# frankyeh/UNet-Studio

Hardware: AMD Instinct MI355X
Metric: voxels/sec 3D U-Net train step @128^3 bf16 (higher is better)
Workload: dtype bf16

## Files before the change

unet-studio_amd/csrc/engine.cpp:

```cpp
#include <hip/hip_runtime.h>

#include <algorithm>
#include <atomic>
#include <cmath>
#include <cstdio>
#include <cstring>
#include <functional>
#include <stdexcept>
#include <string>
#include <mutex>
#include <random>
#include <unordered_map>
#include <vector>

#include "../../include/unet_hip.h"
#include "conv_select.h"
#include "graph.hpp"
#include "kernels.h"

using namespace unet;

namespace {

thread_local std::string g_err;
// ... 729 lines not shown
            const bool defer = gflat && p.wz_job_of_op[i] >= 0 && !on_main;
            const bool own = p.wz_off[i] != SIZE_MAX && (defer || (op.kind == OP_CONV && p.conv[i].wgrad == Wgrad::mfma));
            {
            ProfScope pw(i, UNET_PROF_WGRAD, sb);
            conv_wgrad(p.conv[i].wgrad, op.kind == OP_CONVT, p.dtype, cg, sd, op.nsrc, gptr(t), gparams[op.weight], gparams[op.bias],
                       ws + (own ? p.wz_off[i] : p.wgrad_off), on_main ? s : sb, defer, on_main ? 0 : p.side_polite[i], nullptr);
            }
            if (defer) { wz_ran[p.wz_job_of_op[i]] = 1; ++wz_pending; }
            if (wz_pending >= 3) flush_wz(sb);
        };
        const int64_t hold_from = (int64_t)64 * 64 * 64, hold_below = (int64_t)32 * 32 * 32;
        std::vector<int> held;
        bool deep_seen = false;
        constexpr int fork_every = 3;
        std::vector<int> pending;
        auto issue_pending = [&]() {
            if (pending.empty()) return;
            fork();
            for (int h : pending) do_wgrad(h);
            pending.clear();
        };
        for (int i = (int)g.ops.size() - 1; i >= op_lo; --i) {
            const Op& op = g.ops[i];
            const bool dry = i >= op_hi;
            if (op.kind == OP_NORM) continue;
            if (op.kind == OP_EXPORT) {
                if (grad_outs && grad_outs[op.out_level] && g.tensors[op.src[0]].needs_grad) {
                    if (!dry) launch_export_bwd(p.dtype, grad_outs[op.out_level], dst_of(op.src[0]), g.tensors[op.src[0]].voxels(), s);
                    mark(op);
                }
                continue;
            }
            int t = op.dst;
            if ((op.kind == OP_CONV) && op.out_level >= 0) {
                if (!(grad_outs && grad_outs[op.out_level])) continue;
                if (p.conv[i].fwd == Fwd::head) {
                    DstGrad dgh = dst_of(op.src[0]);
                    ProfScope ph(dry ? -2 : i, UNET_PROF_OTHER, s);
                    if (!dry) {
                        const bool defer = sb != s && p.head_op_off[i] != SIZE_MAX;
                        char* hs = ws + (defer ? p.head_op_off[i] : p.head_off);
                        launch_head_bwd(p.dtype, geom(op), src(op.src[0]), grad_outs[op.out_level], nullptr, params[op.weight], dgh,
                                        gparams[op.weight], gparams[op.bias], hs, s, defer);
                        if (defer) { fork(); launch_head_bwd_reduce(geom(op), gparams[op.weight], gparams[op.bias], hs, sb); }
                    }
                    if (dgh.ptr) mark(op);
                    continue;
                }
                if (!dry) launch_import_grad(p.dtype, grad_outs[op.out_level], gptr(t), g.tensors[t].C, g.tensors[t].voxels(), 0, s);
                init[t] = 1;
            }
            if (!g.tensors[t].needs_grad || !init[t]) continue;
            bool first_fused = false;
            if (!dry && p.conv[i].wgrad == Wgrad::first_mfma && g.tensors[t].norm >= 0 && !g.tensors[op.src[0]].needs_grad && sb != s &&
                p.wz_off[i] != SIZE_MAX && g.tensors[t].C % 8 == 0)
                first_fused = !env().no_first_wgrad_fuse;
            {
                const bool has_norm = g.tensors[t].norm >= 0;
                const bool done = has_norm && norm_done[t];
                int rows = 0;
                if (done) norm_done[t] = 0;
                else if (has_norm) { if (bn_tensor == t) rows = bn_rows; bn_tensor = -1; }
                if (!dry) { ProfScope ps(i, UNET_PROF_NORM_BWD, s); if (!done) view_backward(t, params, gparams, first_fused, rows); }
            }
            switch (op.kind) {
                case OP_CONV:
                case OP_CONVT: {
                    SrcDesc sd[2] = {src(op.src[0]), op.nsrc > 1 ? src(op.src[1]) : SrcDesc()};
                    DstGrad dg[2] = {dst_of(op.src[0]), op.nsrc > 1 ? dst_of(op.src[1]) : DstGrad()};
                    ConvGeom cg = geom(op);
                    const float* wd = (const float*)(ws + p.w_dgrad[i]);
                    bool any = dg[0].ptr || (op.nsrc > 1 && dg[1].ptr);
                    if (!dry && !any && sb != s && p.conv[i].wgrad == Wgrad::first_mfma && p.wz_off[i] != SIZE_MAX) {
                        ProfScope pw(i, UNET_PROF_WGRAD, s);
                        const Tensor& To = g.tensors[t];
                        NormBwdFuse nf = {tptr(t), first_fused ? stat(To.norm) : nullptr, first_fused ? coef(To.norm) : nullptr, To.act};
                        conv_wgrad(p.conv[i].wgrad, false, p.dtype, cg, sd, op.nsrc, gptr(t), gparams[op.weight], gparams[op.bias], ws + p.wz_off[i],
                                   s, false, 0, first_fused ? &nf : nullptr);
                    } else
                    if (!dry) {
                        const int64_t vox = (int64_t)cg.Do * cg.Ho * cg.Wo;
                        if (!deep_seen && vox <= hold_below && !held.empty()) {
                            deep_seen = true;
                            pending.insert(pending.begin(), held.begin(), held.end());
                            held.clear();
                            pending.push_back(i);
                            issue_pending();
                        } else if (!deep_seen && sb != s && vox >= hold_from) held.push_back(i);
                        else {
                            pending.push_back(i);
                            if ((int)pending.size() >= fork_every || sb == s || vox >= hold_below) issue_pending();
                        }
                    }
                    ProfScope pd(i, UNET_PROF_DGRAD, s);
                    if (any) {
                        const int ts = op.src[0];
                        const Tensor& Ts = g.tensors[ts];
                        const bool can = op.nsrc == 1 && Ts.norm >= 0 && p.first_consumer[ts] == i && p.dtype == UNET_DTYPE_BF16;
                        DeepNormBwd nb;
                        if (can) {
                            const Norm& n = g.norms[Ts.norm];
                            nb = {tptr(ts), stat(Ts.norm), params[n.gamma], coef(Ts.norm), gparams[n.gamma], gparams[n.beta], Ts.act};
                        }
                        const DgradOutcome o = conv_dgrad(p.conv[i].dgrad, op.kind == OP_CONVT, p.dtype, cg, gptr(t), at(p.wm_dgrad[i]), wd, dg, op.nsrc,
                                                          can ? &nb : nullptr, partial(), deep(), s, !dry);
                        if (o.norm_done) norm_done[ts] = 1;
                        if (o.rows > 0) { bn_tensor = ts; bn_rows = o.rows; }
                        mark(op);
                    }
                    break;
                }
                case OP_MATERIALIZE: {
                    DstGrad dg[2] = {dst_of(op.src[0]), op.nsrc > 1 ? dst_of(op.src[1]) : DstGrad()};
                    if (dg[0].ptr || (op.nsrc > 1 && dg[1].ptr)) {
                        if (!dry) launch_materialize_bwd(p.dtype, gptr(t), dg, op.nsrc, g.tensors[t].voxels(), s);
                        mark(op);
                    }
                    break;
                }
                case OP_MAXPOOL: {
                    const Tensor& a = g.tensors[op.src[0]];
                    DstGrad d = dst_of(op.src[0]);
                    if (d.ptr) { if (!dry) launch_maxpool_bwd(p.dtype, src(op.src[0]), gptr(t), d, a.D, a.H, a.W, s); mark(op); }
                    break;
                }
                case OP_UPSAMPLE: {
                    const Tensor& a = g.tensors[op.src[0]];
                    DstGrad d = dst_of(op.src[0]);
                    if (d.ptr) { if (!dry) launch_upsample_bwd(p.dtype, gptr(t), d, a.D, a.H, a.W, s); mark(op); }
// ... 1905 lines not shown
```

unet-studio_amd/csrc/kernels.h:

```cpp
#pragma once
#include <hip/hip_runtime.h>
#include <cstdint>

#include "../../include/unet_atlas.h"
#include "../../include/unet_augment.h"
#include "../../include/unet_calib.h"
#include "../../include/unet_recal.h"
#include "../../include/unet_components.h"
#include "../../include/unet_connectivity.h"
#include "../../include/unet_distance.h"
#include "../../include/unet_ensemble.h"
#include "../../include/unet_feed.h"
#include "../../include/unet_hip.h"
#include "../../include/unet_instances.h"
#include "../../include/unet_morph.h"
#include "../../include/unet_postproc.h"
#include "../../include/unet_preproc.h"
#include "../../include/unet_qc.h"
#include "../../include/unet_register.h"
#include "../../include/unet_space.h"
#include "../../include/unet_stats.h"
#include "../../include/unet_table.h"
#include "../../include/unet_mirror.h"
#include "../../include/unet_tiles.h"
// ... 98 lines not shown
                     int* zero, int nzero, const float* partial, int nblk, float lr, float momentum, int nesterov, float weight_decay,
                     float clip_norm, float grad_scale, float* norm_out, hipStream_t s);

struct PackJob { int64_t src_off, dst_off, total, blk0; int Ci, Co, CK, T, mode, A, B, pad; };
enum PackMode {
    PK_CONV_FWD = 0,
    PK_CONV_DGRAD = 1,
    PK_CONVT_DGRAD = 2,
    PK_CONVT_FWD = 3,
    PK_CONV_S2_DGRAD = 4
};
int mfma_conv_pack_jobs(const ConvGeom& g, bool want_dgrad, PackJob* out2);
int mfma_convt_pack_jobs(const ConvGeom& g, PackJob* out2);
void launch_mfma_pack_batched(const float* params_base, void* ws, const PackJob* jobs_dev, int njobs, int64_t nblocks, hipStream_t s,
                              int64_t blk_base = 0, int max_grid = 0, int* zero = nullptr, int nzero = 0);
bool mfma_conv_fwd_supported(int dtype, const ConvGeom& g, const SrcDesc* src, int nsrc);
size_t mfma_conv_w_bytes(const ConvGeom& g);
void launch_mfma_pack_conv_w(const float* w, void* w_mfma_fwd, void* w_mfma_dgrad, const ConvGeom& g, hipStream_t s);
int launch_mfma_conv_fwd(const ConvGeom& g, const SrcDesc* src, int nsrc, const void* w_mfma, const float* bias, void* out,
                         float* stats_partial, hipStream_t s);
bool conv_first_mfma_supported(int dtype, const ConvGeom& g, const SrcDesc* src, int nsrc);
int conv_first_mfma_blocks(const ConvGeom& g);
int launch_conv_first_mfma(const ConvGeom& g, const SrcDesc* src, const float* w, const float* bias, void* out, float* stats_partial,
                           hipStream_t s);
int mfma_conv_blocks(const ConvGeom& g);
bool mfma_wgrad_z_supported(int dtype, const ConvGeom& g, const SrcDesc* src, int nsrc);
size_t mfma_wgrad_z_scratch_bytes(const ConvGeom& g, int polite = 0);
int mfma_wgrad_z_splits(const ConvGeom& g, int polite = 0);
int launch_mfma_wgrad_z(const ConvGeom& g, const SrcDesc* src, int nsrc, const void* dy, bool want_bias, void* scratch, hipStream_t s,
                        int polite = 0);
void wgrad_reduce(const float* slab, const float* bias_slab, int nsplit, int64_t n, int Cb, float* dw, float* db, hipStream_t s);
struct WgradReduceJob { long long slab_off, bias_off, dw_off, db_off, n; int nsplit, Cb, ly, blk0, nblk, op; };
int wgrad_reduce_job_blocks(WgradReduceJob& j, int blk0);
void launch_wgrad_reduce_batched(const WgradReduceJob* jobs_dev, int job0, int njobs, int blk_base, int nblocks, const void* ws, float* gflat,
                                 hipStream_t s);
bool mfma_wgrad_supported(int dtype, const ConvGeom& g, const SrcDesc* src, int nsrc);
size_t mfma_wgrad_scratch_bytes(const ConvGeom& g, int polite = 0);
int mfma_conv_wgrad_splits(const ConvGeom& g, int polite = 0);
int mfma_convt_wgrad_splits(const ConvGeom& g);
bool mfma_conv_wgrad_direct(const ConvGeom& g);
bool mfma_convt_wgrad_direct(const ConvGeom& g);
int conv_first_wgrad_splits(const ConvGeom& g);
void launch_mfma_conv_wgrad(const ConvGeom& g, const SrcDesc* src, int nsrc, const void* dy, float* dw, float* db, void* scratch,
                            hipStream_t s, bool defer_reduce = false, int polite = 0);
bool head_supported(const ConvGeom& g, int nsrc);
size_t head_bwd_scratch_bytes(const ConvGeom& g);
void launch_head_fwd(int dtype, const ConvGeom& g, const SrcDesc& src, const float* w, const float* bias, void* y, float* out_ncdhw,
                     hipStream_t s);
void launch_head_bwd(int dtype, const ConvGeom& g, const SrcDesc& src, const float* dy_ncdhw, const void* dy_cl, const float* w,
                     DstGrad dst, float* dw, float* db, void* scratch, hipStream_t s, bool defer_reduce = false);
void launch_head_bwd_reduce(const ConvGeom& g, float* dw, float* db, const void* scratch, hipStream_t s);
bool conv_first_wgrad_mfma_supported(int dtype, const ConvGeom& g, const SrcDesc* src, int nsrc);
size_t conv_first_wgrad_mfma_scratch_bytes(const ConvGeom& g);
struct NormBwdFuse { const void* u; const float* stat; const float* coef; int act; };
void launch_conv_first_wgrad_mfma(const ConvGeom& g, const SrcDesc* src, const void* dy, float* dw, float* db, void* scratch, hipStream_t s,
                                  bool defer_reduce = false, const NormBwdFuse* nb_fuse = nullptr);
bool wgrad_small_supported(const ConvGeom& g, int nsrc);
size_t wgrad_small_scratch_bytes(const ConvGeom& g);
void launch_conv_wgrad_small(int dtype, const ConvGeom& g, const SrcDesc* src, int nsrc, const void* dy, float* dw, float* db,
                             void* scratch, hipStream_t s);
bool mfma_convt_wgrad_supported(int dtype, const ConvGeom& g, const SrcDesc* src, int nsrc);
size_t mfma_convt_wgrad_scratch_bytes(const ConvGeom& g);
void launch_mfma_convt_wgrad(const ConvGeom& g, const SrcDesc* src, const void* dy, float* dw, void* scratch, hipStream_t s,
                             bool defer_reduce = false, float* db = nullptr, int polite = 0);
int launch_colsum_partial8(int dtype, const void* x, int C, int64_t S, float* partial, hipStream_t s);
size_t bias_grad_scratch_bytes(int C, int64_t S);
void launch_bias_grad(int dtype, const void* dy, int C, int64_t S, float* db, void* scratch, hipStream_t s);
bool mfma_conv_dgrad_supported(int dtype, const ConvGeom& g, const SrcDesc* src, int nsrc);
size_t mfma_conv_dgrad_w_bytes(const ConvGeom& g);
struct DgradOutcome {
    bool served = false;
    bool norm_done = false;
    int rows = 0;
    bool operator==(const DgradOutcome& o) const { return served == o.served && norm_done == o.norm_done && rows == o.rows; }
};
struct BnBwdStats { const void* u; const float* stat; float* partial; int act, C; };
DgradOutcome mfma_conv_dgrad_outcome(const ConvGeom& g, const DstGrad* dst, int ndst, bool norm);
DgradOutcome launch_mfma_conv_dgrad(const ConvGeom& g, const void* dy, const void* w_mfma_dgrad, const DstGrad* dst, int ndst, hipStream_t s,
                                    const BnBwdStats* bn = nullptr);
int launch_s2_conv_fwd(const ConvGeom& g, const SrcDesc* src, int nsrc, const void* w_mfma, const float* bias, void* out, float* stats_partial,
                       hipStream_t s);
DgradOutcome s2_conv_dgrad_outcome(const ConvGeom& g, const DstGrad* dst, int ndst, bool norm);
DgradOutcome launch_s2_conv_dgrad(const ConvGeom& g, const void* dy, const void* w_s2_dgrad, const DstGrad* dst, int ndst, hipStream_t s,
                                  const BnBwdStats* bn);
int s2_conv_dgrad_rows_max();
bool launch_s2_convt_fwd(const ConvGeom& g, const SrcDesc* src, int nsrc, const void* w_mfma, const float* bias, void* out, hipStream_t s);
bool launch_s2_convt_dgrad(const ConvGeom& g, const void* dy, const void* w_mfma_dgrad, const DstGrad* dst, int ndst, hipStream_t s);
int s2_wgrad_splits(int Ca, int Cb, int cD, int cH, int cW);
int launch_s2_wgrad(int ks, const void* fine, const void* fine2, int C0, int Ca, int fD, int fH, int fW, const void* coarse, int Cb, int cD, int cH,
                    int cW, bool want_bias, int bias_from_a, void* scratch, hipStream_t s, int polite);
constexpr int64_t DEEP_MAX_VOXELS = 512;
struct DeepScratch { float* part = nullptr; size_t part_bytes = 0; int* cnt = nullptr; int ncnt = 0; };
struct DeepNormFwd {
    const float* gamma; const float* beta; double eps; float* stat; float* rm; float* rv; double momentum; int use_running; int act;
    void* act_out;
};
struct DeepNormBwd {
    const void* u; const float* stat; const float* gamma; float* coef; float* dgamma; float* dbeta; int act;
};
bool deep_conv_applies(int dtype, int64_t out_voxels, int cin, int cout);
bool launch_deep_conv_fwd(const ConvGeom& g, const SrcDesc* src, int nsrc, const void* w_mfma, const float* bias, void* out,
                          const DeepNormFwd* nf, const DeepScratch& sc, hipStream_t s);
bool launch_deep_convt_fwd(const ConvGeom& g, const SrcDesc* src, int nsrc, const void* w_mfma, const float* bias, void* out,
                           const DeepScratch& sc, hipStream_t s);
DgradOutcome deep_dgrad_outcome(const ConvGeom& g, bool transposed, const DstGrad* dst, int ndst, bool norm, const DeepScratch& sc);
DgradOutcome launch_deep_dgrad(const ConvGeom& g, bool transposed, const void* dy, const void* w_mfma_dgrad, const DstGrad* dst, int ndst,
                               const DeepNormBwd* nb, const DeepScratch& sc, hipStream_t s);
// ... 160 lines not shown
```

unet-studio_amd/csrc/kernels_mfma_conv.hip:

```cpp
#include <type_traits>
#include <cstdlib>
#include "mfma_util.h"

namespace unet {

constexpr int PACK_LDS_ELEMS = 16 * (32 * 27 + 1);
template <int CK, int T, int MODE>
__device__ __forceinline__ void pack_unit_t(const float* __restrict__ w, __bf16* __restrict__ out, int unit, int Co, int A, int B, __bf16* lds) {
    constexpr int KSTEPS = CK == 32 ? T : (T + 1) / 2;
    const int NTT = Co / 16;
    const int q = unit / NTT, nt = unit % NTT, o0 = nt * 16;
    constexpr int RS = CK * T + 1;
    constexpr int n = 16 * CK * T, U = 8;
    for (int e0 = threadIdx.x; e0 < n; e0 += 256 * U) {
        float v[U];
        int dst[U];
#pragma unroll
        for (int u = 0; u < U; ++u) {
            const int e = e0 + u * 256;
            int r = 0, c = 0, t = 0;
            int64_t src = -1;
            if (e < n) {
                if constexpr (MODE == PK_CONV_FWD || MODE == PK_CONVT_DGRAD) {
                    const int Ax = MODE == PK_CONV_FWD ? A : B;
// ... 573 lines not shown
                    const float mean = a.bn_stat[c + r], rstd = a.bn_stat[a.bn_C + c + r];
                    const float dv = rr[r] * act_d(fmaf(uu[r], a.bn_stat[2 * a.bn_C + c + r], a.bn_stat[3 * a.bn_C + c + r]), a.bn_act);
                    s1[r] = dv; s2[r] = dv * ((uu[r] - mean) * rstd);
                }
            } else {
                s1[0] = r0; s1[1] = r1; s1[2] = r2; s1[3] = r3;
                s2[0] = r0 * r0; s2[1] = r1 * r1; s2[2] = r2 * r2; s2[3] = r3 * r3;
            }
        }
    }
    float* const srows = BNS ? a.bn_partial : a.stats;
    if (srows) {
        __syncthreads();
#pragma unroll
        for (int r = 0; r < 4; ++r) {
            float u = s1[r], v = s2[r];
#pragma unroll
            for (int m = 1; m < 16; m <<= 1) { u += __shfl_xor(u, m); v += __shfl_xor(v, m); }
            if (j == 0) { red[(wave * 16 + gq * 4 + r) * 2] = u; red[(wave * 16 + gq * 4 + r) * 2 + 1] = v; }
        }
        __syncthreads();
        if (tid < 16) {
            float u = 0.f, v = 0.f;
#pragma unroll
            for (int w = 0; w < 4; ++w) { u += red[(w * 16 + tid) * 2]; v += red[(w * 16 + tid) * 2 + 1]; }
            srows[((size_t)bid * g.Cout + nt0 * 16 + tid) * 2 + 0] = u;
            srows[((size_t)bid * g.Cout + nt0 * 16 + tid) * 2 + 1] = v;
        }
    }
}

struct ConvFirstArgs {
    ConvGeom g;
    const void* x;
    const float* w;
    const float* bias;
    void* out;
    float* stats;
    int tiles_x, tiles_y, tiles_z;
};
template <int NT>
__global__ void __launch_bounds__(256, 2) k_conv_first_mfma(ConvFirstArgs a) {
    constexpr int BZ = 4, BY = 8, BX = 16, HZ = BZ + 2, HY = BY + 2, HX = BX + 2, NV = HZ * HY * HX;
    constexpr int ITERS = (NV + 255) / 256;
    __shared__ unsigned short tile[NV + 8];
    __shared__ float red[4 * NT * 16 * 2];
    const ConvGeom& g = a.g;
    const int tid = threadIdx.x, wave = tid >> 6, lane = tid & 63, j = lane & 15, gq = lane >> 4;
    const int ntiles = a.tiles_x * a.tiles_y * a.tiles_z;
    const unsigned short* x = (const unsigned short*)a.x;

    bf16x8 wfrag[NT];
#pragma unroll
    for (int n = 0; n < NT; ++n)
#pragma unroll
        for (int e = 0; e < 8; ++e) {
            const int tap = 8 * gq + e;
            wfrag[n][e] = (__bf16)(tap < 27 ? a.w[(n * 16 + j) * 27 + tap] : 0.f);
        }
    int abase[8];
#pragma unroll
    for (int e = 0; e < 8; ++e) {
        const int tap = 8 * gq + e < 27 ? 8 * gq + e : 26;
        abase[e] = ((((tap / 9) + wave) * HY + (tap / 3) % 3) * HX + tap % 3 + j) * 2;
    }
    float b4[NT][4];
#pragma unroll
    for (int n = 0; n < NT; ++n)
#pragma unroll
        for (int r = 0; r < 4; ++r) b4[n][r] = a.bias ? a.bias[n * 16 + gq * 4 + r] : 0.f;
    float s1[NT][4], s2[NT][4];
#pragma unroll
    for (int n = 0; n < NT; ++n)
#pragma unroll
        for (int r = 0; r < 4; ++r) { s1[n][r] = 0.f; s2[n][r] = 0.f; }

    int upk[ITERS];
    unsigned uvox[ITERS];
#pragma unroll
    for (int k = 0; k < ITERS; ++k) {
        const int u = tid + k * 256, hz = u / (HY * HX), hr = u % (HY * HX), hy = hr / HX, hx = hr % HX;
        upk[k] = u < NV ? (hz | (hy << 4) | (hx << 9)) : -1;
        uvox[k] = (unsigned)((hz * g.H + hy) * g.W + hx);
    }
    unsigned short R[ITERS];
    auto prefetch = [&](int t) {
        const int x0 = (t % a.tiles_x) * BX, y0 = ((t / a.tiles_x) % a.tiles_y) * BY, z0 = (t / (a.tiles_x * a.tiles_y)) * BZ;
        const int iz0 = z0 - 1, iy0 = y0 - 1, ix0 = x0 - 1;
        const long long org = ((long long)iz0 * g.H + iy0) * g.W + ix0;
#pragma unroll
        for (int k = 0; k < ITERS; ++k) {
            const int uc = upk[k];
            const int gz = iz0 + (uc & 15), gy = iy0 + ((uc >> 4) & 31), gx = ix0 + ((uc >> 9) & 63);
            R[k] = 0;
            if (uc >= 0 && (unsigned)gz < (unsigned)g.D && (unsigned)gy < (unsigned)g.H && (unsigned)gx < (unsigned)g.W)
                R[k] = x[org + uvox[k]];
        }
    };
    if ((int)blockIdx.x < ntiles) prefetch(blockIdx.x);
    for (int t = blockIdx.x; t < ntiles; t += gridDim.x) {
        __syncthreads();
#pragma unroll
        for (int k = 0; k < ITERS; ++k)
            if (upk[k] >= 0) tile[tid + k * 256] = R[k];
        __syncthreads();
        if (t + (int)gridDim.x < ntiles) prefetch(t + gridDim.x);
        const int x0 = (t % a.tiles_x) * BX, y0 = ((t / a.tiles_x) % a.tiles_y) * BY, z0 = (t / (a.tiles_x * a.tiles_y)) * BZ;
        const int gz = z0 + wave, gx = x0 + j;
#pragma unroll
        for (int i = 0; i < BY; ++i) {
            unsigned d[4];
#pragma unroll
            for (int e = 0; e < 4; ++e) {
                const unsigned lo = *(const unsigned short*)((const char*)tile + abase[2 * e] + i * HX * 2);
                const unsigned hi = *(const unsigned short*)((const char*)tile + abase[2 * e + 1] + i * HX * 2);
                d[e] = lo | (hi << 16);
// ... 561 lines not shown
```

unet-studio_amd/csrc/kernels_mfma_wgrad.hip:

```cpp
#include <type_traits>
#include "mfma_util.h"

namespace unet {

typedef __attribute__((ext_vector_type(4))) short s16x4;
typedef __attribute__((address_space(3))) s16x4 lds_s16x4;

struct MfmaWgradArgs {
    ConvGeom g;
    SrcDesc asrc[2];
    int nasrc;
    SrcDesc bsrc;
    float* slab;
    float* bias_slab;
    int tiles_x, tiles_y, tiles_z;
    int direct;
    int bias_from_a;
};

__device__ __forceinline__ bf16x8 tr_read2(const char* p0, const char* p1) {
    s16x4 a = __builtin_amdgcn_ds_read_tr16_b64_v4i16((lds_s16x4*)p0);
    s16x4 b = __builtin_amdgcn_ds_read_tr16_b64_v4i16((lds_s16x4*)p1);
    return __builtin_bit_cast(bf16x8, __builtin_shufflevector(a, b, 0, 1, 2, 3, 4, 5, 6, 7));
}
// ... 386 lines not shown
    const long long n = jb.n, ntot = n + (hb ? jb.Cb : 0);
    const long long i = ((long long)((int)blockIdx.x + blk_base - jb.blk0) * LX + lx) * 4;
    double s0 = 0.0, s1 = 0.0, s2 = 0.0, s3 = 0.0;
    if (i < ntot) {
        const float* base = i < n ? ws + jb.slab_off + i : ws + jb.bias_off + (i - n);
        const long long stride = i < n ? n : jb.Cb;
        int k = ly;
        for (; k + 7 * LY < jb.nsplit; k += 8 * LY) {
            float4 v[8];
#pragma unroll
            for (int u = 0; u < 8; ++u) v[u] = *(const float4*)(base + (long long)(k + u * LY) * stride);
#pragma unroll
            for (int u = 0; u < 8; ++u) { s0 += v[u].x; s1 += v[u].y; s2 += v[u].z; s3 += v[u].w; }
        }
        for (; k < jb.nsplit; k += LY) {
            const float4 v = *(const float4*)(base + (long long)k * stride);
            s0 += v.x; s1 += v.y; s2 += v.z; s3 += v.w;
        }
    }
    if (LY > 1) {
        red[threadIdx.x][0] = s0; red[threadIdx.x][1] = s1; red[threadIdx.x][2] = s2; red[threadIdx.x][3] = s3;
        __syncthreads();
        if (ly == 0) {
            s0 = s1 = s2 = s3 = 0.0;
            for (int k = 0; k < LY; ++k) { s0 += red[k * LX + lx][0]; s1 += red[k * LX + lx][1]; s2 += red[k * LX + lx][2]; s3 += red[k * LX + lx][3]; }
        }
    }
    if (ly == 0 && i < ntot) {
        float* d = i < n ? gflat + jb.dw_off + i : gflat + jb.db_off + (i - n);
        d[0] += (float)s0; d[1] += (float)s1; d[2] += (float)s2; d[3] += (float)s3;
    }
}
int wgrad_reduce_job_blocks(WgradReduceJob& j, int blk0) {
    j.ly = j.nsplit > 64 ? 16 : (j.nsplit > 8 ? 4 : 1);
    const long long quads = (j.n + (j.bias_off >= 0 ? j.Cb : 0) + 3) / 4;
    const int lx = 256 / j.ly;
    j.blk0 = blk0;
    j.nblk = (int)((quads + lx - 1) / lx);
    return j.nblk;
}
void launch_wgrad_reduce_batched(const WgradReduceJob* jobs_dev, int job0, int njobs, int blk_base, int nblocks, const void* ws, float* gflat,
                                 hipStream_t s) {
    if (njobs <= 0 || nblocks <= 0) return;
    k_wgrad_reduce_batched<<<(unsigned)nblocks, 256, 0, s>>>(jobs_dev, job0, njobs, blk_base, (const float*)ws, gflat);
}

struct FirstWgradArgs {
    ConvGeom g;
    const void* x;
    const void* dy;
    float* slab;
    float* bslab;
    int tiles_x, tiles_y, tiles_z;
    const void* u;
    const float* stat;
    const float* coef;
    int act;
};
template <int NT, bool FUSE>
__global__ void __launch_bounds__(256, 2) k_wgrad_first_mfma(FirstWgradArgs a) {
    constexpr int TZ = 2, TY = 8, TX = 32, HZ = TZ + 2, HY = TY + 2, NROW = TZ * TY, CO = 16 * NT;
    constexpr int XCOPY = HZ * HY * TX;
    constexpr int VSB = CO * 2 + 4;
    constexpr int DY_OFF = 3 * XCOPY * 2;
    __shared__ __attribute__((aligned(16))) char sm[DY_OFF + NROW * TX * VSB + 16];
    const ConvGeom& g = a.g;
    const int tid = threadIdx.x, wave = tid >> 6, lane = tid & 63, j = lane & 15, gq = lane >> 4;
    const unsigned short* x = (const unsigned short*)a.x;
    const char* dyb = (const char*)a.dy;
    int abase[2];
    bool ones_row = false;
#pragma unroll
    for (int rt = 0; rt < 2; ++rt) {
        int tap = rt * 16 + j;
        if (tap == 27) ones_row = true;
        if (tap > 26) tap = 26;
        const int kz = tap / 9, ky = (tap / 3) % 3, kx = tap % 3;
        abase[rt] = (kx * XCOPY + (kz * HY + ky) * TX + gq * 8) * 2;
    }
    const bf16x8 ones = __builtin_bit_cast(bf16x8, make_uint4(0x3f803f80u, 0x3f803f80u, 0x3f803f80u, 0x3f803f80u));
    f32x4 acc[2][NT];
#pragma unroll
    for (int rt = 0; rt < 2; ++rt)
#pragma unroll
        for (int n = 0; n < NT; ++n) acc[rt][n] = f32x4{0.f, 0.f, 0.f, 0.f};
    const int ntiles = a.tiles_x * a.tiles_y * a.tiles_z;
    constexpr int XI = (HZ * HY * (TX + 2) + 255) / 256, DI = NROW * TX * (CO / 8) / 256;
    static_assert(NROW * TX * (CO / 8) % 256 == 0, "dy units per thread");
    unsigned short xr[XI];
    uint4 dr[DI], ur[FUSE ? DI : 1];
    unsigned dmask = 0;
    float cA[8], cB[8], cD[8], csc[8], csh[8];
    if constexpr (FUSE) {
        const int c0 = (tid % (CO / 8)) * 8;
#pragma unroll
        for (int e = 0; e < 8; ++e) {
            const int c = c0 + e;
            const float mean = a.stat[c], rstd = a.stat[CO + c];
            csc[e] = a.stat[2 * CO + c]; csh[e] = a.stat[3 * CO + c];
            cA[e] = a.coef[c];
            cB[e] = -a.coef[c] * rstd * a.coef[2 * CO + c];
            cD[e] = -a.coef[c] * (a.coef[CO + c] - mean * rstd * a.coef[2 * CO + c]);
        }
    }
    const char* ub = (const char*)a.u;
    auto gload = [&](int t) {
        const int x0 = (t % a.tiles_x) * TX, y0 = ((t / a.tiles_x) % a.tiles_y) * TY, z0 = (t / (a.tiles_x * a.tiles_y)) * TZ;
#pragma unroll
        for (int i = 0; i < XI; ++i) {
            const int e = tid + i * 256;
            const int hx = e % (TX + 2), r = e / (TX + 2), hy = r % HY, hz = r / HY;
            const int gz = z0 - 1 + hz, gy = y0 - 1 + hy, gx = x0 - 1 + hx;
            unsigned short v = 0;
            if (e < HZ * HY * (TX + 2) && (unsigned)gz < (unsigned)g.D && (unsigned)gy < (unsigned)g.H && (unsigned)gx < (unsigned)g.W)
                v = x[((size_t)gz * g.H + gy) * g.W + gx];
            xr[i] = v;
        }
#pragma unroll
        for (int i = 0; i < DI; ++i) {
            const int u = tid + i * 256;
            const int c8 = u % (CO / 8), vx = (u / (CO / 8)) % TX, row = u / ((CO / 8) * TX);
            const int gz = z0 + row / TY, gy = y0 + row % TY, gx = x0 + vx;
            uint4 v = make_uint4(0u, 0u, 0u, 0u), w = make_uint4(0u, 0u, 0u, 0u);
            const bool in = gz < g.D && gy < g.H && gx < g.W;
            const size_t off = ((((size_t)gz * g.H + gy) * g.W + gx) * CO + c8 * 8) * 2;
            if (in) v = *(const uint4*)(dyb + off);
            if constexpr (FUSE) {
                if (in) w = *(const uint4*)(ub + off);
                ur[i] = w;
                dmask = in ? (dmask | (1u << i)) : (dmask & ~(1u << i));
            }
            dr[i] = v;
        }
    };
    auto lstore = [&]() {
#pragma unroll
        for (int i = 0; i < XI; ++i) {
            const int e = tid + i * 256;
            if (e < HZ * HY * (TX + 2)) {
                const int hx = e % (TX + 2), r = e / (TX + 2), hy = r % HY, hz = r / HY;
#pragma unroll
                for (int sft = 0; sft < 3; ++sft) {
                    const int k = hx - sft;
                    if (k >= 0 && k < TX) *(unsigned short*)(sm + (sft * XCOPY + (hz * HY + hy) * TX + k) * 2) = xr[i];
                }
            }
        }
#pragma unroll
        for (int i = 0; i < DI; ++i) {
            const int u = tid + i * 256;
            const int c8 = u % (CO / 8), vx = (u / (CO / 8)) % TX, row = u / ((CO / 8) * TX);
            unsigned* d = (unsigned*)(sm + DY_OFF + (row * TX + vx) * VSB + c8 * 16);
            if constexpr (FUSE) {
                if ((dmask >> i) & 1u) {
                    const unsigned gu[4] = {dr[i].x, dr[i].y, dr[i].z, dr[i].w}, uu[4] = {ur[i].x, ur[i].y, ur[i].z, ur[i].w};
                    unsigned o[4];
#pragma unroll
                    for (int e = 0; e < 8; e += 2) {
                        const float g0 = __uint_as_float(gu[e / 2] << 16), g1 = __uint_as_float(gu[e / 2] & 0xffff0000u);
                        const float u0 = __uint_as_float(uu[e / 2] << 16), u1 = __uint_as_float(uu[e / 2] & 0xffff0000u);
                        const float r0 = fmaf(cA[e] * g0, act_d(fmaf(u0, csc[e], csh[e]), a.act), fmaf(cB[e], u0, cD[e]));
                        const float r1 = fmaf(cA[e + 1] * g1, act_d(fmaf(u1, csc[e + 1], csh[e + 1]), a.act), fmaf(cB[e + 1], u1, cD[e + 1]));
                        o[e / 2] = (unsigned)__bfloat16_as_ushort(__float2bfloat16(r0)) | ((unsigned)__bfloat16_as_ushort(__float2bfloat16(r1)) << 16);
                    }
                    dr[i] = make_uint4(o[0], o[1], o[2], o[3]);
                }
            }
            d[0] = dr[i].x; d[1] = dr[i].y; d[2] = dr[i].z; d[3] = dr[i].w;
        }
    };
    if ((int)blockIdx.x < ntiles) gload(blockIdx.x);
    for (int t = blockIdx.x; t < ntiles; t += gridDim.x) {
        __syncthreads();
        lstore();
        __syncthreads();
        if (t + (int)gridDim.x < ntiles) gload(t + gridDim.x);
#pragma unroll 1
        for (int row = wave; row < NROW; row += 4) {
            const int rz = row / TY, ry = row % TY;
            const int roff = (rz * HY + ry) * TX * 2;
            bf16x8 af[2];
#pragma unroll
            for (int rt = 0; rt < 2; ++rt) af[rt] = *(const bf16x8*)(sm + abase[rt] + roff);
            if (ones_row) af[1] = ones;
#pragma unroll
            for (int n = 0; n < NT; ++n) {
                unsigned d[4];
                const char* pb = sm + DY_OFF + (row * TX + gq * 8) * VSB + (n * 16 + j) * 2;
#pragma unroll
                for (int e = 0; e < 4; ++e) {
                    const unsigned lo = *(const unsigned short*)(pb + (2 * e) * VSB), hi = *(const unsigned short*)(pb + (2 * e + 1) * VSB);
                    d[e] = lo | (hi << 16);
                }
                const bf16x8 bf = __builtin_bit_cast(bf16x8, make_uint4(d[0], d[1], d[2], d[3]));
#pragma unroll
                for (int rt = 0; rt < 2; ++rt) acc[rt][n] = __builtin_amdgcn_mfma_f32_16x16x32_bf16(af[rt], bf, acc[rt][n], 0, 0, 0);
            }
        }
    }
    __syncthreads();
    float* red = (float*)sm;
#pragma unroll
    for (int rt = 0; rt < 2; ++rt)
#pragma unroll
        for (int n = 0; n < NT; ++n) *(f32x4*)(red + (((wave * 2 + rt) * NT + n) * 64 + lane) * 4) = acc[rt][n];
    __syncthreads();
    const int O = 27 * g.Cout;
    float* sl = a.slab + (size_t)blockIdx.x * O;
    for (int e = tid; e < 2 * NT * 256; e += 256) {
        float v = 0.f;
#pragma unroll
        for (int w = 0; w < 4; ++w) v += red[w * 2 * NT * 256 + e];
        const int reg = e & 3, l2 = (e >> 2) & 63, rn = e >> 8, n = rn % NT, rt = rn / NT;
        const int tap = rt * 16 + 4 * (l2 >> 4) + reg, co = n * 16 + (l2 & 15);
        if (tap < 27) sl[co * 27 + tap] = v;
        else if (tap == 27) a.bslab[(size_t)blockIdx.x * g.Cout + co] = v;
    }
}
bool conv_first_wgrad_mfma_supported(int dtype, const ConvGeom& g, const SrcDesc* src, int nsrc) {
    return dtype == 1 && nsrc == 1 && g.Cin == 1 && g.ks == 3 && g.stride == 1 && (g.Cout == 16 || g.Cout == 32) && !src[0].scale &&
           src[0].act == 0;
}
static int first_wgrad_blocks(const ConvGeom& g) {
    int tiles = ((g.W + 31) / 32) * ((g.H + 7) / 8) * ((g.D + 1) / 2);
    return tiles < 512 ? tiles : 512;
}
size_t conv_first_wgrad_mfma_scratch_bytes(const ConvGeom& g) { return (size_t)first_wgrad_blocks(g) * (27 * g.Cout + g.Cout) * 4 + 256; }
int conv_first_wgrad_splits(const ConvGeom& g) { return first_wgrad_blocks(g); }
void launch_conv_first_wgrad_mfma(const ConvGeom& g, const SrcDesc* src, const void* dy, float* dw, float* db, void* scratch, hipStream_t s,
                                  bool defer_reduce, const NormBwdFuse* nb_fuse) {
    FirstWgradArgs a;
    a.g = g; a.x = src[0].ptr; a.dy = dy; a.slab = (float*)scratch;
    a.u = nb_fuse ? nb_fuse->u : nullptr; a.stat = nb_fuse ? nb_fuse->stat : nullptr; a.coef = nb_fuse ? nb_fuse->coef : nullptr;
    a.act = nb_fuse ? nb_fuse->act : 0;
    a.tiles_x = (g.W + 31) / 32; a.tiles_y = (g.H + 7) / 8; a.tiles_z = (g.D + 1) / 2;
    const int nb = first_wgrad_blocks(g);
    const int64_t O = 27 * g.Cout;
    a.bslab = a.slab + (size_t)nb * O;
    if (nb_fuse) {
        if (g.Cout == 16) k_wgrad_first_mfma<1, true><<<nb, 256, 0, s>>>(a);
        else k_wgrad_first_mfma<2, true><<<nb, 256, 0, s>>>(a);
    } else {
        if (g.Cout == 16) k_wgrad_first_mfma<1, false><<<nb, 256, 0, s>>>(a);
        else k_wgrad_first_mfma<2, false><<<nb, 256, 0, s>>>(a);
    }
    if (!defer_reduce) wgrad_reduce(a.slab, db ? a.bslab : nullptr, nb, O, g.Cout, dw, db, s);
}

static bool chan16(const ConvGeom& g, const SrcDesc* src, int nsrc) {
    if (g.Cin % 16 || g.Cout % 16) return false;
    for (int s = 0; s < nsrc; ++s)
        if (src[s].C % 16 || src[s].scale || src[s].act) return false;
    return true;
}
bool mfma_wgrad_supported(int dtype, const ConvGeom& g, const SrcDesc* src, int nsrc) {
    return dtype == 1 && g.ks == 3 && (g.stride == 1 || g.stride == 2) && chan16(g, src, nsrc);
}
bool mfma_convt_wgrad_supported(int dtype, const ConvGeom& g, const SrcDesc* src, int nsrc) {
    return dtype == 1 && nsrc == 1 && chan16(g, src, nsrc);
}

struct WgradCfg { int bz, by, bx, pi, pj, nsplit, gy, direct, polite = 0; };
static bool wgrad_direct_cfg(int kind, int bD, int bH, int bW, WgradCfg& c) {
    if (bD != bH || bH != bW) return false;
    if (bW == 4) { c.bz = 4; c.by = 4; c.bx = 4; }
    else if (bW == 8 && kind == 0) { c.bz = 8; c.by = 8; c.bx = 8; }
    else if (bW == 8) { c.bz = 2; c.by = 8; c.bx = 8; }
    else return false;
    c.pi = c.pj = 1; c.nsplit = 1; c.direct = 1;
    return true;
}
static WgradCfg wgrad_cfg(int kind, int Ca, int Cb, int bD, int bH, int bW) {
    WgradCfg c;
    c.direct = 0;
    int cat = Ca / 16, cbt = Cb / 16;
    if (wgrad_direct_cfg(kind, bD, bH, bW, c)) { c.gy = cat * cbt; return c; }
    if (kind == 0) {
        c.pi = cat % 2 == 0 ? 2 : 1; c.pj = cbt % 2 == 0 ? 2 : 1;
        if (bW >= 12) { c.pi = 1; c.pj = 1; }
        if (bW >= 12) { c.bz = 2; c.by = 8; c.bx = 16; }
        else if (bW > 4) { c.bz = 4; c.by = 8; c.bx = 8; }
        else { c.bz = 4; c.by = 8; c.bx = 4; }
    } else {
        c.pi = 1; c.pj = cbt % 4 == 0 ? 4 : (cbt % 2 == 0 ? 2 : 1);
        if (bW >= 12) { c.bz = 2; c.by = 4; c.bx = 16; }
        else if (bW > 4) { c.bz = 2; c.by = 8; c.bx = 8; }
// ... 149 lines not shown
```

unet-studio_amd/csrc/mfma_util.h:

```cpp
#pragma once
#include <atomic>
#include <cstdint>
#include <cstdlib>

#include "device_util.h"

namespace unet {

inline void set_max_lds_once(std::atomic<uint64_t>& done, const void* fn, int bytes) {
    int dev = 0;
    (void)hipGetDevice(&dev);
    const uint64_t bit = 1ull << (dev & 63);
    if (done.load(std::memory_order_acquire) & bit) return;
    (void)hipFuncSetAttribute(fn, hipFuncAttributeMaxDynamicSharedMemorySize, bytes);
    done.fetch_or(bit, std::memory_order_release);
}

inline int polite_lds(int lds, int polite) {
    constexpr int want = 83000;
    return (polite && want > lds) ? want : lds;
}
inline bool sliding_window_off() {
    static const bool off = getenv("UNET_NO_SLIDING_WINDOW") != nullptr;
    return off;
}

typedef __attribute__((ext_vector_type(8))) __bf16 bf16x8;
typedef __attribute__((ext_vector_type(4))) float f32x4;

__device__ __forceinline__ unsigned pack_bf16x2(float lo, float hi) {
    return (unsigned)__bfloat16_as_ushort(__float2bfloat16(lo)) | ((unsigned)__bfloat16_as_ushort(__float2bfloat16(hi)) << 16);
}
__device__ __forceinline__ float bf_lo(unsigned w) { return __uint_as_float(w << 16); }
__device__ __forceinline__ float bf_hi(unsigned w) { return __uint_as_float(w & 0xffff0000u); }

__device__ __forceinline__ int xcd_remap(int b, int n) {
    int q = n >> 3, r = n & 7, x = b & 7;
    return (x < r ? x * (q + 1) : r * (q + 1) + (x - r) * q) + (b >> 3);
}

__device__ __forceinline__ uint4 transform8(uint4 v, bool xf, const float* sc, const float* sh, int act) {
    if (!(xf || act)) return v;
    unsigned wv[4] = {v.x, v.y, v.z, v.w};
#pragma unroll
    for (int e = 0; e < 4; ++e) {
        float lo = bf_lo(wv[e]), hi = bf_hi(wv[e]);
        if (xf) { lo = fmaf(lo, sc[2 * e], sh[2 * e]); hi = fmaf(hi, sc[2 * e + 1], sh[2 * e + 1]); }
        lo = act_f(lo, act); hi = act_f(hi, act);
        wv[e] = pack_bf16x2(lo, hi);
    }
    return make_uint4(wv[0], wv[1], wv[2], wv[3]);
}

struct MfmaConvArgs {
    ConvGeom g;
    SrcDesc src[2];
    int nsrc;
    const void* w;
    const float* bias;
    void* out[2];
    int outC[2];
    int out_acc[2];
    int nout;
    float* stats;
    int tiles_x, tiles_y, tiles_z;
    int sc_C;
    int oD, oH, oW;
    const void* bn_u = nullptr;
    const float* bn_stat = nullptr;
    float* bn_partial = nullptr;
    int bn_act = 0, bn_C = 0;
};

struct ZWork { int nseg, zlen, cols_x, cols_y; };
inline int z_split(ZWork& zw, int planes, int gy, int min_zlen) {
    const int cols = zw.cols_x * zw.cols_y;
    int want = 512 / gy;
    if (want < 1) want = 1;
    const int nseg = (want + cols - 1) / cols;
    int zlen = (planes + nseg - 1) / nseg;
    if (zlen < min_zlen) zlen = min_zlen;
    if (zlen > planes) zlen = planes;
    zw.nseg = (planes + zlen - 1) / zlen; zw.zlen = zlen;
    const int items = cols * zw.nseg;
    return items < want ? items : want;
}
int launch_conv_z16(const MfmaConvArgs& a, hipStream_t s);
// ... 7 lines not shown
```

Baseline: 824.1 million.

## Recompute first-conv pre-norm output inside fused wgrad instead of loading it

The fused first-layer weight-gradient kernel no longer reads the saved pre-normalization activation u from global memory. It recomputes u on the fly from the single-channel input halo already staged in shared memory, using an MFMA with the first conv's weights plus bias, then applies the norm/activation backward before writing dy to LDS. The goal is to cut global memory traffic for a large 128^3 multichannel tensor, paid for with extra MFMA work, more registers and reloaded loads. The fusion is now restricted to layers whose forward also uses the first_mfma path, and a staging structure with masked loads is added, though the stage count is 1.

New measurement: 825.8 million (median of 4 runs). No clear change (+0.2%).

```diff
diff --git a/unet-studio_amd/csrc/engine.cpp b/unet-studio_amd/csrc/engine.cpp
--- a/unet-studio_amd/csrc/engine.cpp
+++ b/unet-studio_amd/csrc/engine.cpp
@@ -805,7 +805,7 @@
             }
             if (!g.tensors[t].needs_grad || !init[t]) continue;
             bool first_fused = false;
-            if (!dry && p.conv[i].wgrad == Wgrad::first_mfma && g.tensors[t].norm >= 0 && !g.tensors[op.src[0]].needs_grad && sb != s &&
+            if (!dry && p.conv[i].wgrad == Wgrad::first_mfma && p.conv[i].fwd == Fwd::first_mfma && g.tensors[t].norm >= 0 && !g.tensors[op.src[0]].needs_grad && sb != s &&
                 p.wz_off[i] != SIZE_MAX && g.tensors[t].C % 8 == 0)
                 first_fused = !env().no_first_wgrad_fuse;
             {
@@ -827,7 +827,7 @@
                     if (!dry && !any && sb != s && p.conv[i].wgrad == Wgrad::first_mfma && p.wz_off[i] != SIZE_MAX) {
                         ProfScope pw(i, UNET_PROF_WGRAD, s);
                         const Tensor& To = g.tensors[t];
-                        NormBwdFuse nf = {tptr(t), first_fused ? stat(To.norm) : nullptr, first_fused ? coef(To.norm) : nullptr, To.act};
+                        NormBwdFuse nf = {params[op.weight], params[op.bias], first_fused ? stat(To.norm) : nullptr, first_fused ? coef(To.norm) : nullptr, To.act};
                         conv_wgrad(p.conv[i].wgrad, false, p.dtype, cg, sd, op.nsrc, gptr(t), gparams[op.weight], gparams[op.bias], ws + p.wz_off[i],
                                    s, false, 0, first_fused ? &nf : nullptr);
                     } else
diff --git a/unet-studio_amd/csrc/kernels.h b/unet-studio_amd/csrc/kernels.h
--- a/unet-studio_amd/csrc/kernels.h
+++ b/unet-studio_amd/csrc/kernels.h
@@ -174,7 +174,7 @@
 void launch_head_bwd_reduce(const ConvGeom& g, float* dw, float* db, const void* scratch, hipStream_t s);
 bool conv_first_wgrad_mfma_supported(int dtype, const ConvGeom& g, const SrcDesc* src, int nsrc);
 size_t conv_first_wgrad_mfma_scratch_bytes(const ConvGeom& g);
-struct NormBwdFuse { const void* u; const float* stat; const float* coef; int act; };
+struct NormBwdFuse { const float* w; const float* bias; const float* stat; const float* coef; int act; };
 void launch_conv_first_wgrad_mfma(const ConvGeom& g, const SrcDesc* src, const void* dy, float* dw, float* db, void* scratch, hipStream_t s,
                                   bool defer_reduce = false, const NormBwdFuse* nb_fuse = nullptr);
 bool wgrad_small_supported(const ConvGeom& g, int nsrc);
diff --git a/unet-studio_amd/csrc/kernels_mfma_conv.hip b/unet-studio_amd/csrc/kernels_mfma_conv.hip
--- a/unet-studio_amd/csrc/kernels_mfma_conv.hip
+++ b/unet-studio_amd/csrc/kernels_mfma_conv.hip
@@ -649,16 +649,11 @@
 
     bf16x8 wfrag[NT];
 #pragma unroll
-    for (int n = 0; n < NT; ++n)
-#pragma unroll
-        for (int e = 0; e < 8; ++e) {
-            const int tap = 8 * gq + e;
-            wfrag[n][e] = (__bf16)(tap < 27 ? a.w[(n * 16 + j) * 27 + tap] : 0.f);
-        }
+    for (int n = 0; n < NT; ++n) wfrag[n] = first_conv_wfrag(a.w, n, j, gq);
     int abase[8];
 #pragma unroll
     for (int e = 0; e < 8; ++e) {
-        const int tap = 8 * gq + e < 27 ? 8 * gq + e : 26;
+        const int tap = first_conv_tap(gq, e);
         abase[e] = ((((tap / 9) + wave) * HY + (tap / 3) % 3) * HX + tap % 3 + j) * 2;
     }
     float b4[NT][4];
diff --git a/unet-studio_amd/csrc/kernels_mfma_wgrad.hip b/unet-studio_amd/csrc/kernels_mfma_wgrad.hip
--- a/unet-studio_amd/csrc/kernels_mfma_wgrad.hip
+++ b/unet-studio_amd/csrc/kernels_mfma_wgrad.hip
@@ -462,11 +462,13 @@
     float* slab;
     float* bslab;
     int tiles_x, tiles_y, tiles_z;
-    const void* u;
+    const float* w;
+    const float* bias;
     const float* stat;
     const float* coef;
     int act;
 };
+constexpr int first_wgrad_stages(int nt, bool fuse) { return 1; }
 template <int NT, bool FUSE>
 __global__ void __launch_bounds__(256, 2) k_wgrad_first_mfma(FirstWgradArgs a) {
     constexpr int TZ = 2, TY = 8, TX = 32, HZ = TZ + 2, HY = TY + 2, NROW = TZ * TY, CO = 16 * NT;
@@ -497,53 +499,89 @@
     const int ntiles = a.tiles_x * a.tiles_y * a.tiles_z;
     constexpr int XI = (HZ * HY * (TX + 2) + 255) / 256, DI = NROW * TX * (CO / 8) / 256;
     static_assert(NROW * TX * (CO / 8) % 256 == 0, "dy units per thread");
-    unsigned short xr[XI];
-    uint4 dr[DI], ur[FUSE ? DI : 1];
-    unsigned dmask = 0;
-    float cA[8], cB[8], cD[8], csc[8], csh[8];
+    constexpr int MT = (NROW / 4) * (TX / 16);
+    constexpr int NST = first_wgrad_stages(NT, FUSE);
+    struct Stage {
+        unsigned short xr[XI];
+        uint4 dr[FUSE ? 1 : DI];
+        uint2 gr[FUSE ? MT * NT : 1];
+        unsigned xmask, dmask;
+    };
+    Stage st[NST];
+    float cA[NT][4], cB[NT][4], cD[NT][4], csc[NT][4], csh[NT][4], b4[NT][4];
+    bf16x8 wfrag[NT];
+    int ubase[8];
     if constexpr (FUSE) {
-        const int c0 = (tid % (CO / 8)) * 8;
+#pragma unroll
+        for (int n = 0; n < NT; ++n) {
+            wfrag[n] = first_conv_wfrag(a.w, n, j, gq);
+#pragma unroll
+            for (int r = 0; r < 4; ++r) {
+                const int c = n * 16 + gq * 4 + r;
+                const float mean = a.stat[c], rstd = a.stat[CO + c];
+                csc[n][r] = a.stat[2 * CO + c]; csh[n][r] = a.stat[3 * CO + c];
+                cA[n][r] = a.coef[c];
+                cB[n][r] = -a.coef[c] * rstd * a.coef[2 * CO + c];
+                cD[n][r] = -a.coef[c] * (a.coef[CO + c] - mean * rstd * a.coef[2 * CO + c]);
+                b4[n][r] = a.bias ? a.bias[c] : 0.f;
+            }
+        }
 #pragma unroll
         for (int e = 0; e < 8; ++e) {
-            const int c = c0 + e;
-            const float mean = a.stat[c], rstd = a.stat[CO + c];
-            csc[e] = a.stat[2 * CO + c]; csh[e] = a.stat[3 * CO + c];
-            cA[e] = a.coef[c];
-            cB[e] = -a.coef[c] * rstd * a.coef[2 * CO + c];
-            cD[e] = -a.coef[c] * (a.coef[CO + c] - mean * rstd * a.coef[2 * CO + c]);
-        }
-    }
-    const char* ub = (const char*)a.u;
-    auto gload = [&](int t) {
+            const int tap = first_conv_tap(gq, e);
+            ubase[e] = ((tap % 3) * XCOPY + ((tap / 9) * HY + (tap / 3) % 3) * TX + j) * 2;
+        }
+    }
+    auto gload = [&](Stage& q, int t) {
+        const bool tv = t < ntiles;
         const int x0 = (t % a.tiles_x) * TX, y0 = ((t / a.tiles_x) % a.tiles_y) * TY, z0 = (t / (a.tiles_x * a.tiles_y)) * TZ;
+        unsigned xm = 0, dm = 0;
 #pragma unroll
         for (int i = 0; i < XI; ++i) {
             const int e = tid + i * 256;
             const int hx = e % (TX + 2), r = e / (TX + 2), hy = r % HY, hz = r / HY;
             const int gz = z0 - 1 + hz, gy = y0 - 1 + hy, gx = x0 - 1 + hx;
-            unsigned short v = 0;
-            if (e < HZ * HY * (TX + 2) && (unsigned)gz < (unsigned)g.D && (unsigned)gy < (unsigned)g.H && (unsigned)gx < (unsigned)g.W)
-                v = x[((size_t)gz * g.H + gy) * g.W + gx];
-            xr[i] = v;
-        }
-#pragma unroll
-        for (int i = 0; i < DI; ++i) {
-            const int u = tid + i * 256;
-            const int c8 = u % (CO / 8), vx = (u / (CO / 8)) % TX, row = u / ((CO / 8) * TX);
-            const int gz = z0 + row / TY, gy = y0 + row % TY, gx = x0 + vx;
-            uint4 v = make_uint4(0u, 0u, 0u, 0u), w = make_uint4(0u, 0u, 0u, 0u);
-            const bool in = gz < g.D && gy < g.H && gx < g.W;
-            const size_t off = ((((size_t)gz * g.H + gy) * g.W + gx) * CO + c8 * 8) * 2;
-            if (in) v = *(const uint4*)(dyb + off);
-            if constexpr (FUSE) {
-                if (in) w = *(const uint4*)(ub + off);
-                ur[i] = w;
-                dmask = in ? (dmask | (1u << i)) : (dmask & ~(1u << i));
-            }
-            dr[i] = v;
-        }
+            const bool in = tv && e < HZ * HY * (TX + 2) && (unsigned)gz < (unsigned)g.D && (unsigned)gy < (unsigned)g.H && (unsigned)gx < (unsigned)g.W;
+            const size_t idx = in ? ((size_t)gz * g.H + gy) * g.W + gx : (size_t)0;
+            q.xr[i] = x[idx];
+            xm |= (in ? 1u : 0u) << i;
+        }
+        if constexpr (FUSE) {
+#pragma unroll
+            for (int m = 0; m < MT; ++m) {
+                const int row = wave + 4 * (m / (TX / 16)), vx = (m % (TX / 16)) * 16 + j;
+                const int gz = z0 + row / TY, gy = y0 + row % TY, gx = x0 + vx;
+                const bool in = tv && gz < g.D && gy < g.H && gx < g.W;
+                const size_t off = in ? ((((size_t)gz * g.H + gy) * g.W + gx) * CO + gq * 4) * 2 : (size_t)0;
+#pragma unroll
+                for (int n = 0; n < NT; ++n) q.gr[m * NT + n] = *(const uint2*)(dyb + off + (in ? n * 32 : 0));
+                dm |= (in ? 1u : 0u) << m;
+            }
+        } else {
+#pragma unroll
+            for (int i = 0; i < DI; ++i) {
+                const int u = tid + i * 256;
+                const int c8 = u % (CO / 8), vx = (u / (CO / 8)) % TX, row = u / ((CO / 8) * TX);
+                const int gz = z0 + row / TY, gy = y0 + row % TY, gx = x0 + vx;
+                const bool in = tv && gz < g.D && gy < g.H && gx < g.W;
+                const size_t off = in ? ((((size_t)gz * g.H + gy) * g.W + gx) * CO + c8 * 8) * 2 : (size_t)0;
+                q.dr[i] = *(const uint4*)(dyb + off);
+                dm |= (in ? 1u : 0u) << i;
+            }
+        }
+        q.xmask = xm; q.dmask = dm;
     };
-    auto lstore = [&]() {
+    auto prep = [&](Stage& q) {
+#pragma unroll
+        for (int i = 0; i < XI; ++i)
+            if (!((q.xmask >> i) & 1u)) q.xr[i] = 0;
+        if constexpr (!FUSE) {
+#pragma unroll
+            for (int i = 0; i < DI; ++i)
+                if (!((q.dmask >> i) & 1u)) q.dr[i] = make_uint4(0u, 0u, 0u, 0u);
+        }
+    };
+    auto lstore = [&](const Stage& q) {
 #pragma unroll
         for (int i = 0; i < XI; ++i) {
             const int e = tid + i * 256;
@@ -552,39 +590,54 @@
 #pragma unroll
                 for (int sft = 0; sft < 3; ++sft) {
                     const int k = hx - sft;
-                    if (k >= 0 && k < TX) *(unsigned short*)(sm + (sft * XCOPY + (hz * HY + hy) * TX + k) * 2) = xr[i];
-                }
-            }
-        }
-#pragma unroll
-        for (int i = 0; i < DI; ++i) {
-            const int u = tid + i * 256;
-            const int c8 = u % (CO / 8), vx = (u / (CO / 8)) % TX, row = u / ((CO / 8) * TX);
-            unsigned* d = (unsigned*)(sm + DY_OFF + (row * TX + vx) * VSB + c8 * 16);
-            if constexpr (FUSE) {
-                if ((dmask >> i) & 1u) {
-                    const unsigned gu[4] = {dr[i].x, dr[i].y, dr[i].z, dr[i].w}, uu[4] = {ur[i].x, ur[i].y, ur[i].z, ur[i].w};
-                    unsigned o[4];
-#pragma unroll
-                    for (int e = 0; e < 8; e += 2) {
-                        const float g0 = __uint_as_float(gu[e / 2] << 16), g1 = __uint_as_float(gu[e / 2] & 0xffff0000u);
-                        const float u0 = __uint_as_float(uu[e / 2] << 16), u1 = __uint_as_float(uu[e / 2] & 0xffff0000u);
-                        const float r0 = fmaf(cA[e] * g0, act_d(fmaf(u0, csc[e], csh[e]), a.act), fmaf(cB[e], u0, cD[e]));
-                        const float r1 = fmaf(cA[e + 1] * g1, act_d(fmaf(u1, csc[e + 1], csh[e + 1]), a.act), fmaf(cB[e + 1], u1, cD[e + 1]));
-                        o[e / 2] = (unsigned)__bfloat16_as_ushort(__float2bfloat16(r0)) | ((unsigned)__bfloat16_as_ushort(__float2bfloat16(r1)) << 16);
-                    }
-                    dr[i] = make_uint4(o[0], o[1], o[2], o[3]);
-                }
-            }
-            d[0] = dr[i].x; d[1] = dr[i].y; d[2] = dr[i].z; d[3] = dr[i].w;
+                    if (k >= 0 && k < TX) *(unsigned short*)(sm + (sft * XCOPY + (hz * HY + hy) * TX + k) * 2) = q.xr[i];
+                }
+            }
+        }
+        if constexpr (!FUSE) {
+#pragma unroll
+            for (int i = 0; i < DI; ++i) {
+                const int u = tid + i * 256;
+                const int c8 = u % (CO / 8), vx = (u / (CO / 8)) % TX, row = u / ((CO / 8) * TX);
+                unsigned* d = (unsigned*)(sm + DY_OFF + (row * TX + vx) * VSB + c8 * 16);
+                d[0] = q.dr[i].x; d[1] = q.dr[i].y; d[2] = q.dr[i].z; d[3] = q.dr[i].w;
+            }
         }
     };
-    if ((int)blockIdx.x < ntiles) gload(blockIdx.x);
-    for (int t = blockIdx.x; t < ntiles; t += gridDim.x) {
-        __syncthreads();
-        lstore();
-        __syncthreads();
-        if (t + (int)gridDim.x < ntiles) gload(t + gridDim.x);
+    auto produce = [&](const Stage& q) {
+#pragma unroll
+        for (int m = 0; m < MT; ++m) {
+            const int row = wave + 4 * (m / (TX / 16)), vx0 = (m % (TX / 16)) * 16;
+            const int poff = (((row / TY) * HY + row % TY) * TX + vx0) * 2;
+            unsigned d[4];
+#pragma unroll
+            for (int e = 0; e < 4; ++e) {
+                const unsigned lo = *(const unsigned short*)(sm + ubase[2 * e] + poff), hi = *(const unsigned short*)(sm + ubase[2 * e + 1] + poff);
+                d[e] = lo | (hi << 16);
+            }
+            const bf16x8 xfrag = __builtin_bit_cast(bf16x8, make_uint4(d[0], d[1], d[2], d[3]));
+            const bool in = (q.dmask >> m) & 1u;
+#pragma unroll
+            for (int n = 0; n < NT; ++n) {
+                const f32x4 uacc = __builtin_amdgcn_mfma_f32_16x16x32_bf16(wfrag[n], xfrag, f32x4{0.f, 0.f, 0.f, 0.f}, 0, 0, 0);
+                const unsigned up[2] = {pack_bf16x2(uacc[0] + b4[n][0], uacc[1] + b4[n][1]), pack_bf16x2(uacc[2] + b4[n][2], uacc[3] + b4[n][3])};
+                const uint2 gv = q.gr[m * NT + n];
+                const unsigned gp[2] = {gv.x, gv.y};
+                unsigned o[2];
+#pragma unroll
+                for (int h = 0; h < 2; ++h) {
+                    const float g0 = bf_lo(gp[h]), g1 = bf_hi(gp[h]), u0 = bf_lo(up[h]), u1 = bf_hi(up[h]);
+                    const int r = 2 * h;
+                    const float r0 = fmaf(cA[n][r] * g0, act_d(fmaf(u0, csc[n][r], csh[n][r]), a.act), fmaf(cB[n][r], u0, cD[n][r]));
+                    const float r1 = fmaf(cA[n][r + 1] * g1, act_d(fmaf(u1, csc[n][r + 1], csh[n][r + 1]), a.act), fmaf(cB[n][r + 1], u1, cD[n][r + 1]));
+                    o[h] = in ? pack_bf16x2(r0, r1) : 0u;
+                }
+                unsigned* dst = (unsigned*)(sm + DY_OFF + (row * TX + vx0 + j) * VSB + (n * 16 + gq * 4) * 2);
+                dst[0] = o[0]; dst[1] = o[1];
+            }
+        }
+    };
+    auto compute = [&]() {
 #pragma unroll 1
         for (int row = wave; row < NROW; row += 4) {
             const int rz = row / TY, ry = row % TY;
@@ -606,6 +659,28 @@
 #pragma unroll
                 for (int rt = 0; rt < 2; ++rt) acc[rt][n] = __builtin_amdgcn_mfma_f32_16x16x32_bf16(af[rt], bf, acc[rt][n], 0, 0, 0);
             }
+        }
+    };
+    const int G = gridDim.x;
+#pragma unroll
+    for (int s = 0; s < NST; ++s) gload(st[s], (int)blockIdx.x + s * G);
+    prep(st[0]);
+    for (int t0 = blockIdx.x; t0 < ntiles; t0 += NST * G) {
+#pragma unroll
+        for (int s = 0; s < NST; ++s) {
+            const int t = t0 + s * G;
+            if (t < ntiles) {
+                __syncthreads();
+                lstore(st[s]);
+                __syncthreads();
+                if constexpr (FUSE) {
+                    produce(st[s]);
+                    __builtin_amdgcn_wave_barrier();
+                }
+            }
+            gload(st[s], t + NST * G);
+            if (t < ntiles) compute();
+            if (t + G < ntiles) prep(st[(s + 1) % NST]);
         }
     }
     __syncthreads();
@@ -641,7 +716,8 @@
                                   bool defer_reduce, const NormBwdFuse* nb_fuse) {
     FirstWgradArgs a;
     a.g = g; a.x = src[0].ptr; a.dy = dy; a.slab = (float*)scratch;
-    a.u = nb_fuse ? nb_fuse->u : nullptr; a.stat = nb_fuse ? nb_fuse->stat : nullptr; a.coef = nb_fuse ? nb_fuse->coef : nullptr;
+    a.w = nb_fuse ? nb_fuse->w : nullptr; a.bias = nb_fuse ? nb_fuse->bias : nullptr;
+    a.stat = nb_fuse ? nb_fuse->stat : nullptr; a.coef = nb_fuse ? nb_fuse->coef : nullptr;
     a.act = nb_fuse ? nb_fuse->act : 0;
     a.tiles_x = (g.W + 31) / 32; a.tiles_y = (g.H + 7) / 8; a.tiles_z = (g.D + 1) / 2;
     const int nb = first_wgrad_blocks(g);
diff --git a/unet-studio_amd/csrc/mfma_util.h b/unet-studio_amd/csrc/mfma_util.h
--- a/unet-studio_amd/csrc/mfma_util.h
+++ b/unet-studio_amd/csrc/mfma_util.h
@@ -33,6 +33,17 @@
 }
 __device__ __forceinline__ float bf_lo(unsigned w) { return __uint_as_float(w << 16); }
 __device__ __forceinline__ float bf_hi(unsigned w) { return __uint_as_float(w & 0xffff0000u); }
+
+__device__ __forceinline__ int first_conv_tap(int gq, int e) { return 8 * gq + e < 27 ? 8 * gq + e : 26; }
+__device__ __forceinline__ bf16x8 first_conv_wfrag(const float* __restrict__ w, int n, int j, int gq) {
+    bf16x8 f;
+#pragma unroll
+    for (int e = 0; e < 8; ++e) {
+        const int tap = 8 * gq + e;
+        f[e] = (__bf16)(tap < 27 ? w[(n * 16 + j) * 27 + tap] : 0.f);
+    }
+    return f;
+}
 
 __device__ __forceinline__ int xcd_remap(int b, int n) {
     int q = n >> 3, r = n & 7, x = b & 7;
```
